# shangzhouye/stereo-visual-slam

Hardware: AMD Instinct MI355X
Metric: stereo keyframes/sec (ORB+match+tri+local-BA), KITTI-00 1241x376 (higher is better)
Workload: dtype u8+f64

## Files before the change

### stereo-visual-slam_amd/csrc/api.hip

```cpp
#include <stdarg.h>
#include <stdlib.h>

#include <algorithm>
#include <cmath>
#include <cfloat>
#include <vector>

#include "se3_device.h"
#include "vslam_internal.h"

#include <mutex>

namespace vslam {

static thread_local char g_err[512] = "";
void set_error(const char* fmt, ...) {
    va_list ap;
    va_start(ap, fmt);
    vsnprintf(g_err, sizeof(g_err), fmt, ap);
    va_end(ap);
}

struct Prof {
    struct Rec { const char* name; int launches; hipEvent_t e0, e1; };
// ... 33 lines not shown
        prof_set_current(((c)->prof && (c)->prof->on) ? (c)->prof : nullptr);               \
    } while (0)

int DevBuf::reserve(size_t need, hipStream_t stream) {
    if (bytes >= need) return VSLAM_OK;
    VS_HIP(hipStreamSynchronize(stream));
    release();
    const size_t want = std::max(need, min_bytes);
    if (hipMalloc((void**)&p, want) != hipSuccess) { p = nullptr; set_error("%s hipMalloc(%zu) failed", name, want); return VSLAM_ERR_HIP; }
    bytes = want; *acct += want;
    return VSLAM_OK;
}
void DevBuf::release() {
    if (p) { (void)hipFree(p); *acct -= bytes; }
    p = nullptr; bytes = 0;
}

struct Arena : Layout {
    struct Upload { void* d; const void* h; size_t bytes; };
    std::vector<Upload> uploads;
    explicit Arena(uint8_t* b = nullptr) : Layout(b) {}
    template <typename T> T* in(const T* h, size_t n) { T* d = take<T>(n); if (base) uploads.push_back({d, h, n * sizeof(T)}); return d; }
};
template <typename F>
static int arena_stage(Ctx* c, F&& layout) {
    Arena a;
    if (int rc = carve(c->stage, c->stream, a, layout)) return rc;
    for (const Arena::Upload& u : a.uploads) VS_HIP(hipMemcpyAsync(u.d, u.h, u.bytes, hipMemcpyHostToDevice, c->stream));
    return VSLAM_OK;
}

static CamParams cam_of(const Ctx* c) {
    CamParams cam;
    cam.fx = c->p.cam[0]; cam.fy = c->p.cam[1]; cam.cx = c->p.cam[2]; cam.cy = c->p.cam[3]; cam.b = c->p.cam[4];
    cam.dmin = c->p.depth_min; cam.dmax = c->p.depth_max; cam.drel = c->p.depth_reliable; cam.row_tol = c->p.stereo_row_tol;
    return cam;
}

template <typename T>
static int dev_alloc(Ctx* c, T** p, size_t n) {
    VS_HIP(hipMalloc((void**)p, n * sizeof(T)));
    c->dev_bytes += n * sizeof(T);
    return VSLAM_OK;
}

struct TuneKey { const char* name; const char* env; int Tuning::*field; int lo, hi; };
static const TuneKey kTuneKeys[] = {
    {"orb_fuse_min", "VSLAM_ORB_FUSE_MIN", &Tuning::orb_fuse_min, 0, 1 << 30},
    {"anms_cap", "VSLAM_ANMS_CAP", &Tuning::anms_cap, 0, 1 << 30},
    {"sgbm_fuse_min", "VSLAM_SGBM_FUSE_MIN", &Tuning::sgbm_fuse_min, 0, 1 << 30},
    {"sgbm_fwd_min", "VSLAM_SGBM_FWD_MIN", &Tuning::sgbm_fwd_min, 0, 1 << 30},
    {"sgbm_fw_rows", "VSLAM_SGBM_FW_ROWS", &Tuning::sgbm_fw_rows, 32, 64},
    {"pose_only_window", "VSLAM_POSE_ONLY_WINDOW", &Tuning::pose_only_window, 0, 1},
    {"ba_resident", "VSLAM_BA_RESIDENT", &Tuning::ba_resident, 0, 1},
    {"pnp_window", "VSLAM_PNP_WINDOW", &Tuning::pnp_window, 0, 1},
    {"ba_adaptive", "VSLAM_BA_ADAPTIVE", &Tuning::ba_adaptive, 0, 1},
    {"ba_lanes", "VSLAM_BA_LANES", &Tuning::ba_lanes, 256, 512},
    {"track_rule", "VSLAM_TRACK_RULE", &Tuning::track_rule, 0, 1},
    {"rectify_form", "VSLAM_RECTIFY_FORM", &Tuning::rectify_form, 0, 1},
};
static int tune_set(Tuning& t, const TuneKey& k, long v) {
    if (v == -1) { t.*(k.field) = -1; return VSLAM_OK; }
    if (v < k.lo || v > k.hi || (k.field == &Tuning::sgbm_fw_rows && v != 32 && v != 64) || (k.field == &Tuning::ba_lanes && v != 256 && v != 512)) {
        set_error("tuning value %s = %ld out of range (%d..%d%s, or -1 = default)", k.name, v, k.lo, k.hi, k.field == &Tuning::sgbm_fw_rows ? ", 32 or 64" : "");
        return VSLAM_ERR_ARG;
    }
    t.*(k.field) = (int)v;
    return VSLAM_OK;
}
static int tune_from_env(Tuning& t) {
    for (const TuneKey& k : kTuneKeys) {
        const char* e = getenv(k.env);
        if (!e || !*e) continue;
        char* end = nullptr;
        const long v = strtol(e, &end, 10);
        if (end == e || *end != 0) { set_error("environment variable %s = \"%s\" is not an integer", k.env, e); return VSLAM_ERR_ARG; }
        int rc = tune_set(t, k, v);
        if (rc) return rc;
    }
    return VSLAM_OK;
}

static int orb_status_check(Ctx* c, int B) {
    std::vector<int32_t> st(B);
    VS_HIP(hipMemcpyAsync(st.data(), c->orb.d_status, sizeof(int32_t) * B, hipMemcpyDeviceToHost, c->stream));
    VS_HIP(hipStreamSynchronize(c->stream));
    for (int b = 0; b < B; ++b)
        if (st[b]) { set_error("ORB capacity exceeded on image %d (status bits 0x%x)", b, st[b]); return VSLAM_ERR_CAPACITY; }
    return VSLAM_OK;
}

constexpr int kOrbFuseMinDefault = 96;
static int orb_fuse_min(const Ctx* c) { return c->tune.orb_fuse_min >= 0 ? c->tune.orb_fuse_min : kOrbFuseMinDefault; }

static int orb_pipeline(Ctx* c, const uint8_t* d_imgs, size_t img_bytes, int pitch, int B, int anms_num, int regroup, bool describe,
                        vslam_keypoint* d_kps, uint8_t* d_desc, int32_t* d_count) {
    if (B <= 0) return VSLAM_OK;
    if (B > c->p.max_batch) { set_error("batch %d exceeds context max_batch %d", B, c->p.max_batch); return VSLAM_ERR_ARG; }
    int rc;
    const bool fused = describe && B >= orb_fuse_min(c);
    if (fused) {
        if ((rc = launch_orb_pyrblur(c->plan, c->tab, d_imgs, img_bytes, pitch, B, c->orb.d_pyr, c->orb.d_blur, c->p.fast_threshold, c->orb.d_corners,
                                     c->orb.d_corner_cnt, c->orb.d_status, c->stream))) return rc;
    } else {
        if ((rc = launch_orb_pyramid(c->plan, c->tab, d_imgs, img_bytes, pitch, B, c->orb.d_pyr, c->stream))) return rc;
        if ((rc = launch_orb_fast(c->plan, d_imgs, img_bytes, pitch, B, c->orb.d_pyr, c->p.fast_threshold, c->orb.d_corners,
                                  c->orb.d_corner_cnt, c->orb.d_status, c->stream))) return rc;
    }
    if ((rc = launch_orb_select(c->plan, d_imgs, img_bytes, pitch, B, c->orb.d_pyr, c->orb.d_corners, c->orb.d_corner_cnt, c->orb.d_sel,
                                c->orb.d_sel_cnt, c->orb.d_status, c->stream))) return rc;
    if ((rc = launch_orb_anms(c->plan, B, c->orb.d_sel, c->orb.d_sel_cnt, c->plan.sel_cap, anms_num, regroup, d_kps, nullptr, c->orb.d_order, c->p.kp_capacity,
                              d_count, c->orb.d_status, c->orb.d_rad, c->tune.anms_cap, c->orb.d_anms_path, c->stream))) return rc;
    if ((rc = launch_orb_orient(c->plan, d_imgs, img_bytes, pitch, B, c->orb.d_pyr, d_kps, c->orb.d_cs, c->orb.d_order, c->p.kp_capacity, d_count, c->stream))) return rc;
    if (describe) {
        if (!fused && (rc = launch_orb_blur(c->plan, d_imgs, img_bytes, pitch, B, c->orb.d_pyr, c->orb.d_blur, c->stream))) return rc;
        if ((rc = launch_orb_describe(c->plan, d_imgs, img_bytes, pitch, B, c->orb.d_pyr, c->orb.d_blur, d_kps, c->orb.d_cs, c->orb.d_order, c->p.kp_capacity, d_count,
// ... 1408 lines not shown
```

### stereo-visual-slam_amd/csrc/lm_kernels.hip

```cpp
#include "vslam_internal.h"

#include <stdlib.h>

#include <vector>

#include "se3_device.h"
#include "lm_device.h"

namespace vslam {

constexpr int kLmBlock = 512;
constexpr int kLmItemFixed = 128;
constexpr int kLmMinWaves = 2;
constexpr int kLmWaves = kLmBlock / 64;
constexpr int kMaxKf = VSLAM_MAX_KF;
constexpr int kMaxNp = 6 * kMaxKf;
constexpr int kMaxPairs = kMaxKf * (kMaxKf + 1) / 2;
constexpr int kHitsPerEdge = (kMaxKf + 1) / 2 + 1;
constexpr int kDinvLds = 1950;
constexpr int kLin = 2;
constexpr int kPoseParts = 3;
constexpr int kCntStride = 80;
constexpr int kItemSlots = (kMaxPairs + kLmWaves - 1) / kLmWaves;
constexpr int kDbgSlots = 24;
// ... 1219 lines not shown
        while (again) {
            double x[6], E[7], Tt[7], Rtt[12], Hd[36], gd[6];
            const bool ok2 = chol6_solve(H, lambda, g, x);
            if (!ok2) {
#pragma unroll
                for (int i = 0; i < 6; ++i) x[i] = 0;
            }
            se3::exp(x, E);
            se3::mul(E, T, Tt);
            expand_pose(Tt, Rtt);
            double tempChi = evaluate(Rtt, false, Hd, gd);
            if (!ok2) tempChi = 1.7976931348623157e308;
            double scale = 1e-3;
#pragma unroll
            for (int i = 0; i < 6; ++i) scale += x[i] * (lambda * x[i] + g[i]);
            rho_gain = (currentChi - tempChi) / scale;
            if (rho_gain > 0 && isfinite(tempChi)) {
                double alpha = 1. - pow(2 * rho_gain - 1, 3);
                alpha = fmin(alpha, 2. / 3.);
                lambda *= fmax(1. / 3., alpha);
                ni = 2;
                currentChi = tempChi;
#pragma unroll
                for (int i = 0; i < 7; ++i) T[i] = Tt[i];
#pragma unroll
                for (int i = 0; i < 12; ++i) Rt[i] = Rtt[i];
            } else {
                lambda *= ni;
                ni *= 2;
            }
            ++qmax;
            again = (rho_gain < 0) && qmax < 10;
        }
        total_trials += qmax;
        if (st && lane == 0 && it < VSLAM_LM_MAX_ITERS) { st->chi2_iter[it] = currentChi; st->lambda_iter[it] = lambda; st->trials_iter[it] = qmax; }
        if (qmax == 10 || rho_gain == 0) { ++it; break; }
    }
    if (st && lane == 0) { st->iterations = it; st->total_trials = total_trials; st->chi2_final = currentChi; st->lambda_final = lambda; }
    if (lane < 7) d_T[7 * (size_t)b + lane] = T[lane];
    int mine = 0;
    for (int i = lane; i < n; i += 64) {
        const size_t gi = (size_t)b * capacity + i;
        double X, Y, Z, ex, ey;
        project_err(Rt, K, (double)px[3 * i], (double)px[3 * i + 1], (double)px[3 * i + 2], uv[2 * gi], uv[2 * gi + 1], X, Y, Z, ex, ey);
        const double c = ex * ex + ey * ey;
        const bool ok = isfinite(c) && c <= thr2;
        if (inlier) inlier[gi] = ok;
        mine += ok;
    }
    for (int o = 32; o > 0; o >>= 1) mine += __shfl_xor(mine, o);
    if (lane == 0 && n_inl) n_inl[b] = mine;
}

constexpr int kPoBlock = 64 * kMaxKf;
struct PoShared {
    double H[2][kMaxKf][36], g[2][kMaxKf][6];
    double part[2][kMaxKf], spart[2][kMaxKf];
    int cnt[kMaxKf][kMaxKf];
    int kbeg[kMaxKf + 1];
    int flag[2];
    int cin[2][kMaxKf], cout[2][kMaxKf];
    double T[2][kMaxKf][7], R[3][kMaxKf][12];
};
__global__ __launch_bounds__(kPoBlock) void pose_only_wave_kernel(LmKernelArgs ka, int iters, int update_poses) {
    const LmWindowArgs& a = ka.a;
    __shared__ PoShared sm;
    const int w = ka.order ? ka.order[blockIdx.x] : (int)blockIdx.x, tid = threadIdx.x, lane = tid & 63;
    const int wave = __builtin_amdgcn_readfirstlane(tid >> 6);
    if (ka.status[w] != VSLAM_OK) return;
    long long* cyc = ka.dbg_cycles ? ka.dbg_cycles + kDbgSlots * (size_t)w : nullptr;
    long long t_ph = cyc ? clock64() : 0;
#define POH(i) do { if (cyc && tid == 0) { const long long t1__ = clock64(); cyc[i] += t1__ - t_ph; t_ph = t1__; } } while (0)
    const int nk = a.n_kf_w ? min(max(a.n_kf_w[w], 1), a.n_kf) : a.n_kf;
    const int lm0 = a.lm_off[w], e0 = a.edge_off[w], ne = a.edge_off[w + 1] - e0;
    const int32_t* kfi = a.kf_idx + e0;
    const int32_t* lmi = a.lm_idx + e0;
    const float2* uv2 = reinterpret_cast<const float2*>(a.uv) + e0;
    const float* xyz = a.xyz + 3 * (size_t)lm0;
    uint8_t* inl = a.lm_inlier + lm0;
    int32_t* list = a.kf_edges + e0;
    float2* uvk = reinterpret_cast<float2*>(ka.uvk) + e0;
    float4* posk = reinterpret_cast<float4*>(a.lin) + e0;
    double* chik = ka.chi2k + e0;
    const double K[4] = {a.K[0], a.K[1], a.K[2], a.K[3]};
    const CamK ck = make_camk(K);
    const double delta = a.huber_delta;
    const unsigned long long lt_mask = (1ull << lane) - 1ull;
    const int per = (((ne + kMaxKf - 1) / kMaxKf) + 63) & ~63;
    const int c0 = min(wave * per, ne), c1 = min(c0 + per, ne);
    {
        int cnt[kMaxKf];
#pragma unroll
        for (int k = 0; k < kMaxKf; ++k) cnt[k] = 0;
        for (int base = c0; base < c1; base += 256) {
            int kq[4], lq[4]; bool vq[4]; uint8_t iq[4];
#pragma unroll
            for (int u = 0; u < 4; ++u) { const int e = base + 64 * u + lane; vq[u] = e < c1; const int es = min(e, ne - 1); kq[u] = kfi[es]; lq[u] = lmi[es]; }
#pragma unroll
            for (int u = 0; u < 4; ++u) iq[u] = inl[lq[u]];
#pragma unroll
            for (int u = 0; u < 4; ++u) {
                const bool act = vq[u] && iq[u] != 0;
#pragma unroll
                for (int kk = 0; kk < kMaxKf; ++kk) cnt[kk] += __popcll(__ballot(act && kq[u] == kk));
            }
        }
        if (lane < kMaxKf) {
            int v = 0;
#pragma unroll
            for (int kk = 0; kk < kMaxKf; ++kk) if (lane == kk) v = cnt[kk];
            sm.cnt[wave][lane] = v;
        }
        if (tid < 2) sm.flag[tid] = 0;
    }
    __syncthreads();
    int off[kMaxKf];
    {
        int run = 0;
#pragma unroll
        for (int k = 0; k < kMaxKf; ++k) {
            int before = 0, tot = 0;
#pragma unroll
            for (int c = 0; c < kMaxKf; ++c) { const int v = sm.cnt[c][k]; tot += v; if (c < wave) before += v; }
            off[k] = run + before;
            if (tid == 0) sm.kbeg[k] = run;
            run += tot;
        }
        if (tid == 0) sm.kbeg[kMaxKf] = run;
    }
    for (int base = c0; base < c1; base += 256) {
        int kq[4], lq[4], eq[4]; bool vq[4]; uint8_t iq[4]; float2 zq[4]; float Xq[4], Yq[4], Zq[4];
#pragma unroll
        for (int u = 0; u < 4; ++u) {
            const int e = base + 64 * u + lane; vq[u] = e < c1; eq[u] = e;
            const int es = min(e, ne - 1);
            kq[u] = kfi[es]; lq[u] = lmi[es]; zq[u] = uv2[es];
        }
#pragma unroll
        for (int u = 0; u < 4; ++u) { iq[u] = inl[lq[u]]; Xq[u] = xyz[3 * lq[u]]; Yq[u] = xyz[3 * lq[u] + 1]; Zq[u] = xyz[3 * lq[u] + 2]; }
#pragma unroll
        for (int u = 0; u < 4; ++u) {
            const bool act = vq[u] && iq[u] != 0;
#pragma unroll
            for (int kk = 0; kk < kMaxKf; ++kk) {
                const unsigned long long m = __ballot(act && kq[u] == kk);
                if (act && kq[u] == kk) {
                    const int pos = off[kk] + __popcll(m & lt_mask);
                    list[pos] = eq[u]; uvk[pos] = zq[u]; posk[pos] = make_float4(Xq[u], Yq[u], Zq[u], 0.f);
                }
                off[kk] += __popcll(m);
            }
        }
    }
    __syncthreads();
    POH(0);
    const int ntot = sm.kbeg[kMaxKf];
    const bool mine = wave < nk;
    const int kb = mine ? sm.kbeg[wave] : 0, ke = mine ? sm.kbeg[wave + 1] : 0;
    {
        double T[7], Rt[12];
#pragma unroll
        for (int i = 0; i < 7; ++i) T[i] = a.T[((size_t)w * a.n_kf + min(wave, nk - 1)) * 7 + i];
        expand_pose(T, Rt);
        if (lane == 0) {
#pragma unroll
            for (int i = 0; i < 7; ++i) sm.T[0][wave][i] = T[i];
#pragma unroll
            for (int i = 0; i < 12; ++i) { sm.R[0][wave][i] = Rt[i]; sm.R[2][wave][i] = Rt[i]; }
        }
        __builtin_amdgcn_wave_barrier();
    }
    const int slot27 = wave_slot<27>(lane);
    auto evaluate = [&](const double* Rlds, bool lin, int buf, bool store_chi) -> double {
        double R[12];
#pragma unroll
        for (int i = 0; i < 12; ++i) R[i] = uniform_f64(Rlds[i]);
        double part = 0, acc[27];
#pragma unroll
        for (int i = 0; i < 27; ++i) acc[i] = 0;
        float4 pp[2], pn[2]; float2 zz[2], zn[2];
#pragma unroll
        for (int u = 0; u < 2; ++u) { const int j = min(kb + 64 * u + lane, max(ke - 1, 0)); pp[u] = posk[j]; zz[u] = uvk[j]; }
        for (int j0 = kb; j0 < ke; j0 += 128) {
#pragma unroll
            for (int u = 0; u < 2; ++u) { const int j = min(j0 + 128 + 64 * u + lane, ke - 1); pn[u] = posk[j]; zn[u] = uvk[j]; }
#pragma unroll
            for (int u = 0; u < 2; ++u) {
                const int j = j0 + 64 * u + lane;
                if (j >= ke) continue;
                double x, y, ri, wgt, ex, ey, c, rho;
                cam_norm(R, (double)pp[u].x, (double)pp[u].y, (double)pp[u].z, x, y, ri);
                eval_obs(ck, x, y, zz[u], delta, ex, ey, c, rho, wgt);
                part += rho;
                if (store_chi) chik[j] = c;
                if (lin) {
                    double A[12], wA[12];
                    jac_norm(x, y, ri, A);
                    const double l0 = wgt * ck.fx2, l1 = wgt * ck.fy2;
#pragma unroll
                    for (int i = 0; i < 6; ++i) { wA[i] = l0 * A[i]; wA[6 + i] = l1 * A[6 + i]; }
                    int idx = 0;
#pragma unroll
                    for (int r = 0; r < 6; ++r)
#pragma unroll
                        for (int cc = r; cc < 6; ++cc) { acc[idx] = a_fma_pair(wA, r, A, cc, acc[idx]); ++idx; }
#pragma unroll
                    for (int r = 0; r < 6; ++r) acc[21 + r] = a_fma2(wA, r, -ex, -ey, acc[21 + r]);
                }
            }
#pragma unroll
            for (int u = 0; u < 2; ++u) { pp[u] = pn[u]; zz[u] = zn[u]; }
        }
        const double total = wave_sum(part);
        if (lin && mine) {
            wave_reduce_scatter<27>(acc, lane);
            if (slot27 >= 0 && slot27 < 21) {
                int r = 0, rem = slot27;
                while (rem >= 6 - r) { rem -= 6 - r; ++r; }
                const int cc = r + rem;
                sm.H[buf][wave][6 * r + cc] = acc[0]; sm.H[buf][wave][6 * cc + r] = acc[0];
            } else if (slot27 >= 21) sm.g[buf][wave][slot27 - 21] = acc[0];
        }
        return total;
    };
    auto sum_kf = [&](const double* v) -> double {
        double t = 0;
        for (int k = 0; k < nk; ++k) t += v[k];
        return t;
    };
    vslam_lm_stats* st = a.stats ? a.stats + w : nullptr;
    double lambda = 0, ni = 2, currentChi = 0;
    int pc = 0;
    int cur = 0, it = 0, total_trials = 0, pb = 0, fb = 0;
    if (iters > 0) {
        const double c = evaluate(sm.R[pc][wave], true, cur, false);
        if (lane == 0 && mine) sm.part[pb][wave] = c;
        __syncthreads();
        currentChi = sum_kf(sm.part[pb]);
        pb ^= 1;
        double md = 0;
        for (int k = 0; k < nk; ++k)
#pragma unroll
            for (int d = 0; d < 6; ++d) md = fmax(md, fabs(sm.H[cur][k][7 * d]));
        lambda = 1e-5 * md;
        if (st && tid == 0) st->chi2_init = currentChi;
    }
    POH(1);
    for (it = 0; it < iters; ++it) {
        double rho_gain = 0;
        int qmax = 0;
        bool again = true;
        while (again) {
            double x[6] = {0, 0, 0, 0, 0, 0};
            if (mine) {
                double Hk[36], gk[6];
#pragma unroll
                for (int i = 0; i < 36; ++i) Hk[i] = sm.H[cur][wave][i];
#pragma unroll
                for (int i = 0; i < 6; ++i) gk[i] = sm.g[cur][wave][i];
                if (!chol6_solve(Hk, lambda, gk, x) && lane == 0) sm.flag[fb] = 1;
            }
            POH(2);
            __syncthreads();
            POH(3);
            const bool ok2 = sm.flag[fb] == 0;
            if (tid == 0) sm.flag[fb ^ 1] = 0;
            fb ^= 1;
            if (!ok2) {
#pragma unroll
                for (int i = 0; i < 6; ++i) x[i] = 0;
            }
            {
                double E[7], Tc[7], Tt[7], Rtt[12];
#pragma unroll
                for (int i = 0; i < 7; ++i) Tc[i] = sm.T[pc][wave][i];
                se3::exp(x, E);
                se3::mul(E, Tc, Tt);
                expand_pose(Tt, Rtt);
                __builtin_amdgcn_wave_barrier();
                if (lane == 0) {
#pragma unroll
                    for (int i = 0; i < 7; ++i) sm.T[pc ^ 1][wave][i] = Tt[i];
#pragma unroll
                    for (int i = 0; i < 12; ++i) { sm.R[pc ^ 1][wave][i] = Rtt[i]; sm.R[2][wave][i] = Rtt[i]; }
                }
                __builtin_amdgcn_wave_barrier();
            }
            POH(4);
            const double c = evaluate(sm.R[pc ^ 1][wave], true, cur ^ 1, false);
            POH(5);
            double sc = 0;
            if (mine) {
#pragma unroll
                for (int i = 0; i < 6; ++i) sc += x[i] * (lambda * x[i] + sm.g[cur][wave][i]);
            }
            if (lane == 0 && mine) { sm.part[pb][wave] = c; sm.spart[pb][wave] = sc; }
            __syncthreads();
            POH(6);
            double tempChi = sum_kf(sm.part[pb]);
            const double scale = sum_kf(sm.spart[pb]) + 1e-3;
            pb ^= 1;
            if (!ok2) tempChi = 1.7976931348623157e308;
            rho_gain = (currentChi - tempChi) / scale;
            if (rho_gain > 0 && isfinite(tempChi)) {
                double alpha = 1. - pow(2 * rho_gain - 1, 3);
                alpha = fmin(alpha, 2. / 3.);
                lambda *= fmax(1. / 3., alpha);
                ni = 2;
                currentChi = tempChi;
                pc ^= 1;
                cur ^= 1;
            } else {
                lambda *= ni;
                ni *= 2;
            }
            ++qmax;
            again = (rho_gain < 0) && qmax < 10;
        }
        total_trials += qmax;
        if (st && tid == 0 && it < VSLAM_LM_MAX_ITERS) { st->chi2_iter[it] = currentChi; st->lambda_iter[it] = lambda; st->trials_iter[it] = qmax; }
        if (qmax == 10 || rho_gain == 0) { ++it; break; }
    }
    if (st && tid == 0) { st->iterations = it; st->total_trials = total_trials; st->chi2_final = currentChi; st->lambda_final = lambda; }
    POH(7);
    evaluate(sm.R[2][wave], false, 0, true);
    double th = delta;
    int cb = 0;
    for (int iteration = 0; iteration < 5; ++iteration) {
        int cin = 0, cout = 0;
        for (int j = kb + lane; j < ke; j += 64) { if (chik[j] > th) ++cout; else ++cin; }
        for (int o = 32; o > 0; o >>= 1) { cin += __shfl_xor(cin, o); cout += __shfl_xor(cout, o); }
        if (lane == 0) { sm.cin[cb][wave] = mine ? cin : 0; sm.cout[cb][wave] = mine ? cout : 0; }
        __syncthreads();
        int tin = 0, tout = 0;
        for (int k = 0; k < nk; ++k) { tin += sm.cin[cb][k]; tout += sm.cout[cb][k]; }
        cb ^= 1;
        const double ratio = (double)tin / (double)(tin + tout);
        if (ratio > 0.5) break;
        th *= 2;
    }
    if (ka.want_chi2) {
        double* chi2 = a.chi2 + e0;
        for (int e = tid; e < ne; e += kPoBlock) if (!inl[lmi[e]]) chi2[e] = 0.0;
        for (int j = kb + lane; j < ke; j += 64) chi2[list[j]] = chik[j];
    }
    __syncthreads();
    for (int j = kb + lane; j < ke; j += 64) {
        const int e = list[j];
        if (e == ne - 1 || lmi[e + 1] != lmi[e]) inl[lmi[e]] = !(chik[j] > th);
    }
    if (tid == 0 && a.chi2_thr) a.chi2_thr[w] = th;
    if (update_poses && mine && lane < 7) a.T[((size_t)w * a.n_kf + wave) * 7 + lane] = sm.T[pc][wave][lane];
    POH(8);
    (void)ntot;
#undef POH
}

static int carve_lm(LmScratch& s, LmKernelArgs& ka, size_t total_lm, size_t total_edge, int n_windows, bool with_lm, hipStream_t stream) {
    int32_t* defer;
    if (int rc = carve(s.buf, stream, [&](Layout& L) {
            ka.a.P = L.take<double>(total_lm * 3);
            ka.a.Ptrial = L.take<double>(total_lm * 3);
            ka.a.Hll = L.take<double>(total_lm * 6);
            ka.a.bl = L.take<double>(total_lm * 3);
            ka.a.Dinv = L.take<double>(total_lm * 6);
            ka.a.lin = L.take<double>(total_edge * kLin);
            ka.a.lm_ptr = L.take<int32_t>(total_lm + n_windows + 1);
            ka.a.kf_ptr = L.take<int32_t>((size_t)n_windows * (kMaxKf + 1));
            ka.a.kf_edges = L.take<int32_t>(total_edge);
            ka.a.pair_ptr = L.take<int32_t>((size_t)n_windows * (kMaxPairs + 1));
            ka.a.pair_hits = L.take<int32_t>(with_lm ? total_edge * kHitsPerEdge * 2 : 64);
            ka.act = L.take<uint8_t>(total_lm);
            ka.kf_pos = L.take<int32_t>(total_edge);
            ka.status = L.take<int32_t>(n_windows);
            double* chi2 = L.take<double>(total_edge);
            if (!ka.a.chi2) ka.a.chi2 = chi2;
            ka.chi2k = L.take<double>(total_edge);
            ka.uvk = L.take<float>(total_edge * 2);
            ka.slot_uv = L.take<float>(with_lm ? total_lm * kLmSlots * 2 : 64);
            ka.slot_kf = L.take<uint8_t>(with_lm ? total_lm * kLmSlots : 256);
            ka.lcnt = L.take<uint8_t>(total_lm);
            ka.order = L.take<int32_t>(n_windows);
            ka.passes = L.take<int32_t>(n_windows);
            defer = L.take<int32_t>(n_windows);
        })) return rc;
    s.status = ka.status; s.status_n = n_windows; s.passes = ka.passes; s.defer = defer;
    return VSLAM_OK;
}

__global__ void lm_fill_kernel(int32_t* __restrict__ p, int n, int v) { const int i = blockIdx.x * blockDim.x + threadIdx.x; if (i < n) p[i] = v; }
constexpr int kOrderCap = 4096;
__global__ __launch_bounds__(1024) void lm_order_kernel(const int32_t* __restrict__ edge_off, int n, int32_t* __restrict__ order) {
    __shared__ unsigned long long key[kOrderCap];
    int np2 = 1;
    while (np2 < n) np2 <<= 1;
    for (int i = threadIdx.x; i < np2; i += 1024)
        key[i] = i < n ? ((unsigned long long)(0xFFFFFFFFu - (unsigned)max(edge_off[i + 1] - edge_off[i], 0)) << 32) | (unsigned)i : ~0ull;
    for (int k = 2; k <= np2; k <<= 1)
        for (int j = k >> 1; j > 0; j >>= 1) {
            __syncthreads();
            for (int t = threadIdx.x; t < np2 / 2; t += 1024) {
                const int lo = ((t / j) * 2 * j) + (t % j), hi = lo + j;
                const bool up = (lo & k) == 0;
                const unsigned long long x = key[lo], y = key[hi];
                if ((x > y) == up) { key[lo] = y; key[hi] = x; }
            }
        }
// ... 24 lines not shown
        ka.dbg_cycles = (long long*)scratch->cyc.p;
    }
    int rc = carve_lm(*scratch, ka, total_lm, total_edge, a.n_windows, true, stream);
    if (rc) return rc;
    const bool adaptive = !(scratch->tune && scratch->tune->ba_adaptive == 0);
    const bool resident_on = (schedule || mode == 0) && !(scratch->tune && scratch->tune->ba_resident == 0);
    ProfScope prof__(stream, "lm_window_kernel", (schedule ? (adaptive ? 2 : 4) : 1) + (resident_on ? 1 : 0));
    if (a.n_windows > 1 && a.n_windows <= kOrderCap)
        hipLaunchKernelGGL(lm_order_kernel, dim3(1), dim3(1024), 0, stream, a.edge_off, a.n_windows, const_cast<int32_t*>(ka.order));
    else ka.order = nullptr;
    const bool resident = (schedule || mode == 0) && !(scratch->tune && scratch->tune->ba_resident == 0);
    scratch->defer_valid = resident;
    if (resident) {
        if (scratch->rs_dyn_bytes < 0) { int dev = 0; VS_HIP(hipGetDevice(&dev)); rs_query_device(dev, *scratch); }
        RsLaunch L;
        memset(&L, 0, sizeof(L));
        L.a = ka.a; L.uv_s = ka.uvk; L.epos = ka.kf_pos; L.tab = ka.a.Hll; L.xin = ka.a.Ptrial; L.Pbak = ka.a.P; L.Dc = ka.a.Dinv; L.blc = ka.a.bl;
        L.status = ka.status; L.passes = ka.passes; L.defer = scratch->defer; L.order = ka.order; L.dbg = getenv("VSLAM_RS_PROFILE") ? ka.dbg_cycles : nullptr;
        L.lanes = (scratch->tune && scratch->tune->ba_lanes > 0) ? scratch->tune->ba_lanes : 0;
        L.dyn_bytes = scratch->rs_dyn_bytes; L.full_bytes = scratch->rs_full_bytes; L.cu_count = scratch->rs_cu_count; L.schedule = schedule; L.adaptive = adaptive ? 1 : 0; L.iters = iters; L.update_poses = update_poses; L.update_lms = update_lms;
        L.opt_in_done = scratch->rs_opt_in; L.want_chi2 = ka.want_chi2;
        L.dense_to_general = !(scratch->tune && scratch->tune->ba_resident == 1);
        if (schedule && !adaptive) hipLaunchKernelGGL(lm_fill_kernel, dim3((a.n_windows + 255) / 256), dim3(256), 0, stream, ka.passes, a.n_windows, 3);
        rc = launch_ba_resident(L, stream);
        if (rc) return rc;
        scratch->rs_opt_in = true;
        ka.defer = scratch->defer;
        if (L.dbg) {
            hipStreamSynchronize(stream);
            std::vector<long long> h(kDbgSlots * (size_t)a.n_windows);
            hipMemcpy(h.data(), ka.dbg_cycles, sizeof(long long) * h.size(), hipMemcpyDeviceToHost);
            static const char* rs_names[16] = {"setup", "pass init", "boot evaluation", "lambda-init pass", "linearise", "convert+cholesky+solve", "pose update+backsub+trial eval",
                                               "(loop tail)", "classification", "write-back", "lin: row open", "lin: landmark blocks", "lin: diag pair (row-wise)", "lin: off-diag pairs (row-wise)", "lin: singles chunks", "(classification: row loop)"};
            double tot = 0;
            for (int i = 0; i < 16; ++i) { double sum = 0; for (int w = 0; w < a.n_windows; ++w) sum += (double)h[16 * (size_t)w + i]; sum /= a.n_windows; if (i < 10) tot += sum; fprintf(stderr, "  [rs profile] %-32s %10.0f ticks/window\n", rs_names[i], sum); }
            fprintf(stderr, "  [rs profile] total %.0f (clock64 ticks)\n", tot);
            hipMemsetAsync(ka.dbg_cycles, 0, sizeof(long long) * kDbgSlots * a.n_windows, stream);
        }
    }
    if (schedule) {
        if (adaptive) {
            hipLaunchKernelGGL((lm_window_kernel<false, true>), dim3(a.n_windows), dim3(kLmBlock), dyn_lds, stream, ka, 0, 5, 0, 0, 1, 0);
        } else {
            if (!resident) hipLaunchKernelGGL(lm_fill_kernel, dim3((a.n_windows + 255) / 256), dim3(256), 0, stream, ka.passes, a.n_windows, 3);
            hipLaunchKernelGGL(lm_window_kernel<false>, dim3(a.n_windows), dim3(kLmBlock), dyn_lds, stream, ka, 0, 5, 0, 0, 1, 0);
            hipLaunchKernelGGL(lm_window_kernel<false>, dim3(a.n_windows), dim3(kLmBlock), dyn_lds, stream, ka, 0, 5, 0, 0, 1, 1);
            hipLaunchKernelGGL(lm_window_kernel<false>, dim3(a.n_windows), dim3(kLmBlock), dyn_lds, stream, ka, 0, kSchedFinalIters, 1, 0, 1, 1);
        }
        ka.defer = nullptr;
        const bool po_window = scratch->tune && scratch->tune->pose_only_window > 0;
        if (po_window) hipLaunchKernelGGL(lm_window_kernel<false>, dim3(a.n_windows), dim3(kLmBlock), dyn_lds, stream, ka, 1, 10, 1, 0, 1, resident ? 0 : 1);
        else {
            if (ka.dbg_cycles && getenv("VSLAM_PO_PROFILE")) hipMemsetAsync(ka.dbg_cycles, 0, sizeof(long long) * kDbgSlots * a.n_windows, stream);
            hipLaunchKernelGGL(pose_only_wave_kernel, dim3(a.n_windows), dim3(kPoBlock), 0, stream, ka, 10, 1);
        }
    } else {
        hipLaunchKernelGGL(lm_window_kernel<false>, dim3(a.n_windows), dim3(kLmBlock), dyn_lds, stream, ka, mode, iters, update_poses, update_lms, 1, 0);
    }
    VS_HIP(hipGetLastError());
    if (ka.dbg_cycles) {
        hipStreamSynchronize(stream);
        std::vector<long long> h(kDbgSlots * (size_t)a.n_windows);
        hipMemcpy(h.data(), ka.dbg_cycles, sizeof(long long) * h.size(), hipMemcpyDeviceToHost);
        static const char* names[kDbgSlots] = {"setup", "eval+lin", "lm blocks", "pose blocks", "lambda/Dinv", "bs", "schur", "cholesky (rest)", "solve (rest)", "update+scale", "eval trial", "loop tail", "classify+wb", "(setup: csr)", "(setup: kf-major)", "schur: item prologue",
                                               "chol: diag+rows", "chol: barrier 1", "chol: trailing update", "chol: barrier 2", "solve: barrier", "solve: back-subst", "schur: rows", "schur: reduce+store"};
        double tot = 0;
        for (int i = 0; i < kDbgSlots; ++i) { double s = 0; for (int w = 0; w < a.n_windows; ++w) s += (double)h[kDbgSlots * (size_t)w + i]; s /= a.n_windows; if (i < 13 || i >= 16) tot += s; fprintf(stderr, "  [lm profile] %-20s %10.0f ticks/window\n", names[i], s); }
        fprintf(stderr, "  [lm profile] total %.0f cycles (clock64 = shader clock, thread 0 of every window; setup sub-splits not included)\n", tot);
    }
    return VSLAM_OK;
}

int lm_fetch_deferred(const LmScratch* scratch, int n_windows, int32_t* h_defer, hipStream_t stream) {
    if (!scratch->buf.p || !scratch->defer || !h_defer || n_windows > scratch->status_n) return VSLAM_ERR_ARG;
    if (!scratch->defer_valid) { for (int w = 0; w < n_windows; ++w) h_defer[w] = 1; return VSLAM_OK; }
    VS_HIP(hipMemcpyAsync(h_defer, scratch->defer, sizeof(int32_t) * n_windows, hipMemcpyDeviceToHost, stream));
    VS_HIP(hipStreamSynchronize(stream));
    for (int w = 0; w < n_windows; ++w) h_defer[w] &= 1;
    return VSLAM_OK;
}

int lm_fetch_passes(const LmScratch* scratch, int n_windows, int32_t* h_passes, hipStream_t stream) {
    if (!scratch->buf.p || !scratch->passes || !h_passes || n_windows > scratch->status_n) return VSLAM_ERR_ARG;
    VS_HIP(hipMemcpyAsync(h_passes, scratch->passes, sizeof(int32_t) * n_windows, hipMemcpyDeviceToHost, stream));
    VS_HIP(hipStreamSynchronize(stream));
    return VSLAM_OK;
}

int lm_fetch_status(const LmScratch* scratch, int n_windows, int32_t* h_status, hipStream_t stream) {
    const LmScratch& g_lm = *scratch;
    if (!g_lm.buf.p || !h_status) return VSLAM_ERR_ARG;
    VS_HIP(hipMemcpyAsync(h_status, g_lm.status, sizeof(int32_t) * n_windows, hipMemcpyDeviceToHost, stream));
    VS_HIP(hipStreamSynchronize(stream));
    return VSLAM_OK;
}

__global__ __launch_bounds__(256) void edge_jacobian_kernel(int n, const float* __restrict__ xyz, const float* __restrict__ uv, const double* __restrict__ T, double K0, double K1,
                                                           double K2, double K3, double delta, double* __restrict__ err, double* __restrict__ Jp, double* __restrict__ Jl,
                                                           double* __restrict__ chi2, double* __restrict__ hw) {
    const int i = blockIdx.x * 256 + threadIdx.x;
    if (i >= n) return;
    const double K[4] = {K0, K1, K2, K3};
    const CamK ck = make_camk(K);
    double Tl[7], Rt[12];
#pragma unroll
    for (int c = 0; c < 7; ++c) Tl[c] = T[c];
    expand_pose(Tl, Rt);
// ... 54 lines not shown
```

### stereo-visual-slam_amd/csrc/vslam_internal.h

```cpp
#pragma once
#include <hip/hip_runtime.h>
#include <stdint.h>
#include <stdio.h>
#include <string.h>

#include "../../include/vslam_hip.h"

namespace vslam {

void set_error(const char* fmt, ...);

#define VS_HIP(call)                                                                              \
    do {                                                                                          \
        hipError_t e__ = (call);                                                                  \
        if (e__ != hipSuccess) {                                                                  \
            ::vslam::set_error("%s:%d %s -> %s", __FILE__, __LINE__, #call, hipGetErrorString(e__)); \
            return VSLAM_ERR_HIP;                                                                 \
        }                                                                                         \
    } while (0)

struct Prof;
Prof* prof_current();
void prof_set_current(Prof* p);
void prof_begin(hipStream_t s, const char* name, int launches);
// ... 129 lines not shown
                 const int32_t* d_nt, const double* d_gap, int gate, double ratio, double gap_thr, int B, int max_rows,
                 uint32_t* d_train_best, vslam_dmatch* d_out, int out_capacity, int32_t* d_nout, hipStream_t stream,
                 const int32_t* d_qsel = nullptr, int sel_cap = 0, const int32_t* d_nqsel = nullptr, const int32_t* d_qitem = nullptr, int n_qitems = 0);

struct CamParams { double fx, fy, cx, cy, b, dmin, dmax, drel, row_tol; };
int launch_find3d_disparity(const vslam_keypoint* d_kps, int n, const float* d_disp, int w, int h, int dstride,
                            const double* d_T, CamParams cam, float* d_xyz, uint8_t* d_valid, uint8_t* d_rel, hipStream_t stream);
int launch_find3d_disparity_batch(const vslam_keypoint* d_kps, const int32_t* d_n, int kp_capacity, int B, const float* d_disp, int w, int h,
                                  const double* d_T, CamParams cam, float* d_xyz, uint8_t* d_valid, uint8_t* d_rel, hipStream_t stream);
int launch_triangulate(const float* d_uvL, const float* d_uvR, const int32_t* d_n, int capacity, int B, const double* d_T,
                       CamParams cam, float* d_xyz, uint8_t* d_valid, uint8_t* d_rel, hipStream_t stream);
int launch_build_pnp_inputs(const vslam_dmatch* d_m, const int32_t* d_nm, int match_capacity, const vslam_dmatch* d_lr,
                            const int32_t* d_nlr, int lr_capacity, const float* d_xyz_lr, const uint8_t* d_valid_lr,
                            const vslam_keypoint* d_kpsT, int kp_capacity, int B, int32_t* d_kp2lr, float* d_xyz_out, float* d_uv_out,
                            int32_t* d_nout, int out_capacity, hipStream_t stream);
int launch_gather_uv(const vslam_keypoint* d_kpsQ, const vslam_keypoint* d_kpsT, int kp_capacity, const vslam_dmatch* d_m,
                     const int32_t* d_nm, int match_capacity, int B, float* d_uvQ, float* d_uvT, hipStream_t stream);

int launch_hbm_copy_probe(const void* src, void* dst, size_t bytes, int variant, hipStream_t stream);
int hbm_copy_probe_variants();
const char* hbm_copy_probe_name(int variant);

struct LmWindowArgs {
    int n_windows, n_kf;
    const int32_t* n_kf_w;
    const int32_t* lm_off;
    const int32_t* edge_off;
    double* T;
    float* xyz;
    const uint8_t* reliable;
    uint8_t* lm_inlier;
    const int32_t* kf_idx;
    const int32_t* lm_idx;
    const float* uv;
    double* chi2;
    vslam_lm_stats* stats;
    double* P;
    double* Ptrial;
    double* Hll;
    double* bl;
    double* Dinv;
    double* lin;
    int32_t* lm_ptr;
    int32_t* kf_ptr;
    int32_t* kf_edges;
    int32_t* pair_ptr;
    int32_t* pair_hits;
    int32_t hit_capacity_per_edge;
    double K[4];
    double huber_delta;
    double* chi2_thr;
    size_t total_lm, total_edge;
};
struct Tuning {
    int orb_fuse_min = -1;
    int anms_cap = -1;
    int sgbm_fuse_min = -1;
    int sgbm_fwd_min = -1;
    int sgbm_fw_rows = -1;
    int pose_only_window = -1;
    int pnp_window = -1;
    int ba_lanes = -1;
    int ba_resident = -1;
    int track_rule = -1;
    int rectify_form = -1;
    int ba_adaptive = -1;
};
constexpr int kSgbmTicketPools = 8;
constexpr int kSgbmErrorWord = kSgbmTicketPools;
int launch_sgbm(const Tuning& tune, const vslam_sgbm_params& sp, const uint8_t* d_left, const uint8_t* d_right, size_t img_bytes, int pitch, int w, int h, int B,
                float* d_disp_f32, int16_t* d_disp_i16, int16_t* d_disp_raw, DevBuf& scratch, hipStream_t stream);

struct LmScratch {
    DevBuf buf, cyc;
    int32_t* status = nullptr; int status_n = 0;
    int32_t* passes = nullptr;
    const Tuning* tune = nullptr;
    bool lds_opt_in = false;
    bool rs_opt_in = false;
    int rs_dyn_bytes = -1, rs_full_bytes = 0, rs_cu_count = 0;
    int32_t* defer = nullptr;
    bool defer_valid = false;
    explicit LmScratch(size_t* acct) : buf("LM scratch", acct), cyc("LM clock buffer", acct) {}
};
struct RsLaunch {
    LmWindowArgs a;
    void* uv_s; int32_t* epos; double* tab; double* xin; double* Pbak; double* Dc; double* blc;
    int32_t* status; int32_t* passes; int32_t* defer; const int32_t* order; long long* dbg;
    int dyn_bytes, full_bytes, cu_count;
    int schedule, adaptive, iters, update_poses, update_lms, dense_to_general;
    int want_chi2;
    int lanes;
    bool opt_in_done;
};
void rs_query_device(int device, LmScratch& s);
int launch_ba_resident(const RsLaunch& L, hipStream_t stream);
int launch_lm_windows(const LmWindowArgs& a, int schedule, int mode, int iters, int update_poses, int update_lms, LmScratch* scratch,
                      hipStream_t stream);
size_t lm_hits_per_edge();
int lm_fetch_status(const LmScratch* scratch, int n_windows, int32_t* h_status, hipStream_t stream);
int lm_fetch_passes(const LmScratch* scratch, int n_windows, int32_t* h_passes, hipStream_t stream);
int lm_fetch_deferred(const LmScratch* scratch, int n_windows, int32_t* h_defer, hipStream_t stream);

struct PnpArgs {
    const float* xyz; const float* uv; const int32_t* n; int capacity; int B;
    double* T; int iters; double K[4]; double huber_delta; double reproj_thr;
    uint8_t* inlier; int32_t* n_inliers; vslam_lm_stats* stats;
    int n_hint;
};
int launch_pnp(const PnpArgs& a, LmScratch* scratch, hipStream_t stream);
int launch_edge_jacobians(int n, const float* d_xyz, const float* d_uv, const double* d_T, const double K[4], double delta, double* d_err, double* d_Jp, double* d_Jl,
                          double* d_chi2, double* d_hw, hipStream_t stream);
size_t pnp_epnp_ws_bytes(int H);
// ... 61 lines not shown
```

Measured before the change: 64550.

## Add narrow pose-only kernel variant packing several keyframes per wave

The pose-only refinement kernel is templated on the wave count, so one block can run with fewer waves than keyframes. When a block has fewer waves, keyframes are dealt greedily by edge count, and each wave loops over its held keyframes. Solved steps pass through shared memory between waves. The host picks the narrow four-wave variant when there are more windows than CUs, which aims to raise occupancy and cut idle waves, at the cost of serialising work inside each wave. The wide variant also gets a min-waves launch bound of 3.

```diff
diff --git a/stereo-visual-slam_amd/csrc/api.hip b/stereo-visual-slam_amd/csrc/api.hip
--- a/stereo-visual-slam_amd/csrc/api.hip
+++ b/stereo-visual-slam_amd/csrc/api.hip
@@ -109,6 +109,7 @@
     {"sgbm_fwd_min", "VSLAM_SGBM_FWD_MIN", &Tuning::sgbm_fwd_min, 0, 1 << 30},
     {"sgbm_fw_rows", "VSLAM_SGBM_FW_ROWS", &Tuning::sgbm_fw_rows, 32, 64},
     {"pose_only_window", "VSLAM_POSE_ONLY_WINDOW", &Tuning::pose_only_window, 0, 1},
+    {"pose_only_waves", "VSLAM_POSE_ONLY_WAVES", &Tuning::pose_only_waves, 0, VSLAM_MAX_KF},
     {"ba_resident", "VSLAM_BA_RESIDENT", &Tuning::ba_resident, 0, 1},
     {"pnp_window", "VSLAM_PNP_WINDOW", &Tuning::pnp_window, 0, 1},
     {"ba_adaptive", "VSLAM_BA_ADAPTIVE", &Tuning::ba_adaptive, 0, 1},
@@ -118,7 +119,8 @@
 };
 static int tune_set(Tuning& t, const TuneKey& k, long v) {
     if (v == -1) { t.*(k.field) = -1; return VSLAM_OK; }
-    if (v < k.lo || v > k.hi || (k.field == &Tuning::sgbm_fw_rows && v != 32 && v != 64) || (k.field == &Tuning::ba_lanes && v != 256 && v != 512)) {
+    if (v < k.lo || v > k.hi || (k.field == &Tuning::sgbm_fw_rows && v != 32 && v != 64) || (k.field == &Tuning::ba_lanes && v != 256 && v != 512) ||
+        (k.field == &Tuning::pose_only_waves && v != 0 && v != VSLAM_MAX_KF && v != kPoseOnlyNarrowWaves)) {
         set_error("tuning value %s = %ld out of range (%d..%d%s, or -1 = default)", k.name, v, k.lo, k.hi, k.field == &Tuning::sgbm_fw_rows ? ", 32 or 64" : "");
         return VSLAM_ERR_ARG;
     }
diff --git a/stereo-visual-slam_amd/csrc/lm_kernels.hip b/stereo-visual-slam_amd/csrc/lm_kernels.hip
--- a/stereo-visual-slam_amd/csrc/lm_kernels.hip
+++ b/stereo-visual-slam_amd/csrc/lm_kernels.hip
@@ -1295,17 +1295,20 @@
     if (lane == 0 && n_inl) n_inl[b] = mine;
 }
 
-constexpr int kPoBlock = 64 * kMaxKf;
 struct PoShared {
     double H[2][kMaxKf][36], g[2][kMaxKf][6];
     double part[2][kMaxKf], spart[2][kMaxKf];
+    double x[kMaxKf][6];
     int cnt[kMaxKf][kMaxKf];
     int kbeg[kMaxKf + 1];
     int flag[2];
     int cin[2][kMaxKf], cout[2][kMaxKf];
     double T[2][kMaxKf][7], R[3][kMaxKf][12];
 };
-__global__ __launch_bounds__(kPoBlock) void pose_only_wave_kernel(LmKernelArgs ka, int iters, int update_poses) {
+template <int W, int kMinWaves>
+__global__ __launch_bounds__(64 * W, kMinWaves) void pose_only_wave_kernel(LmKernelArgs ka, int iters, int update_poses) {
+    static_assert(W == kMaxKf || (W >= 1 && W <= 8), "the keyframe deal takes its minimum over eight lanes");
+    constexpr int kBlock = 64 * W;
     const LmWindowArgs& a = ka.a;
     __shared__ PoShared sm;
     const int w = ka.order ? ka.order[blockIdx.x] : (int)blockIdx.x, tid = threadIdx.x, lane = tid & 63;
@@ -1329,7 +1332,7 @@
     const CamK ck = make_camk(K);
     const double delta = a.huber_delta;
     const unsigned long long lt_mask = (1ull << lane) - 1ull;
-    const int per = (((ne + kMaxKf - 1) / kMaxKf) + 63) & ~63;
+    const int per = (((ne + W - 1) / W) + 63) & ~63;
     const int c0 = min(wave * per, ne), c1 = min(c0 + per, ne);
     {
         int cnt[kMaxKf];
@@ -1364,7 +1367,7 @@
         for (int k = 0; k < kMaxKf; ++k) {
             int before = 0, tot = 0;
 #pragma unroll
-            for (int c = 0; c < kMaxKf; ++c) { const int v = sm.cnt[c][k]; tot += v; if (c < wave) before += v; }
+            for (int c = 0; c < W; ++c) { const int v = sm.cnt[c][k]; tot += v; if (c < wave) before += v; }
             off[k] = run + before;
             if (tid == 0) sm.kbeg[k] = run;
             run += tot;
@@ -1397,24 +1400,44 @@
     }
     __syncthreads();
     POH(0);
-    const int ntot = sm.kbeg[kMaxKf];
-    const bool mine = wave < nk;
-    const int kb = mine ? sm.kbeg[wave] : 0, ke = mine ? sm.kbeg[wave + 1] : 0;
-    {
+    unsigned long long held = 0;
+    int nheld = 0;
+    if constexpr (W == kMaxKf) { held = (unsigned long long)wave; nheld = wave < nk ? 1 : 0; }
+    else {
+        const int kl = min(lane, kMaxKf - 1);
+        const int mycnt = lane < nk ? sm.kbeg[kl + 1] - sm.kbeg[kl] : -1;
+        int rank = 0;
+        for (int j = 0; j < nk; ++j) { const int cj = sm.kbeg[j + 1] - sm.kbeg[j]; rank += (cj > mycnt || (cj == mycnt && j < lane)) ? 1 : 0; }
+        int load = 0;
+        for (int r = 0; r < nk; ++r) {
+            const int k = __builtin_amdgcn_readfirstlane(__ffsll((long long)__ballot(lane < nk && rank == r)) - 1);
+            const int cr = __shfl(mycnt, k);
+            int key = lane < W ? load * 16 + lane : 0x7fffffff;
+            key = min(key, __shfl_xor(key, 1)); key = min(key, __shfl_xor(key, 2)); key = min(key, __shfl_xor(key, 4));
+            const int v = __builtin_amdgcn_readfirstlane(key) & 15;
+            if (lane == v) load += cr;
+            if (v == wave) { held |= (unsigned long long)k << (4 * nheld); ++nheld; }
+        }
+    }
+    auto kf_at = [&](int q) -> int { return (int)((held >> (4 * q)) & 15ull); };
+#pragma unroll 1
+    for (int q = 0; q < nheld; ++q) {
+        const int k = kf_at(q);
         double T[7], Rt[12];
 #pragma unroll
-        for (int i = 0; i < 7; ++i) T[i] = a.T[((size_t)w * a.n_kf + min(wave, nk - 1)) * 7 + i];
+        for (int i = 0; i < 7; ++i) T[i] = a.T[((size_t)w * a.n_kf + k) * 7 + i];
         expand_pose(T, Rt);
         if (lane == 0) {
 #pragma unroll
-            for (int i = 0; i < 7; ++i) sm.T[0][wave][i] = T[i];
-#pragma unroll
-            for (int i = 0; i < 12; ++i) { sm.R[0][wave][i] = Rt[i]; sm.R[2][wave][i] = Rt[i]; }
-        }
-        __builtin_amdgcn_wave_barrier();
-    }
+            for (int i = 0; i < 7; ++i) sm.T[0][k][i] = T[i];
+#pragma unroll
+            for (int i = 0; i < 12; ++i) { sm.R[0][k][i] = Rt[i]; sm.R[2][k][i] = Rt[i]; }
+        }
+    }
+    __builtin_amdgcn_wave_barrier();
     const int slot27 = wave_slot<27>(lane);
-    auto evaluate = [&](const double* Rlds, bool lin, int buf, bool store_chi) -> double {
+    auto evaluate = [&](const double* Rlds, bool lin, int buf, bool store_chi, int k) -> double {
+        const int kb = __builtin_amdgcn_readfirstlane(sm.kbeg[k]), ke = __builtin_amdgcn_readfirstlane(sm.kbeg[k + 1]);
         double R[12];
 #pragma unroll
         for (int i = 0; i < 12; ++i) R[i] = uniform_f64(Rlds[i]);
@@ -1455,14 +1478,14 @@
             for (int u = 0; u < 2; ++u) { pp[u] = pn[u]; zz[u] = zn[u]; }
         }
         const double total = wave_sum(part);
-        if (lin && mine) {
+        if (lin) {
             wave_reduce_scatter<27>(acc, lane);
             if (slot27 >= 0 && slot27 < 21) {
                 int r = 0, rem = slot27;
                 while (rem >= 6 - r) { rem -= 6 - r; ++r; }
                 const int cc = r + rem;
-                sm.H[buf][wave][6 * r + cc] = acc[0]; sm.H[buf][wave][6 * cc + r] = acc[0];
-            } else if (slot27 >= 21) sm.g[buf][wave][slot27 - 21] = acc[0];
+                sm.H[buf][k][6 * r + cc] = acc[0]; sm.H[buf][k][6 * cc + r] = acc[0];
+            } else if (slot27 >= 21) sm.g[buf][k][slot27 - 21] = acc[0];
         }
         return total;
     };
@@ -1476,8 +1499,12 @@
     int pc = 0;
     int cur = 0, it = 0, total_trials = 0, pb = 0, fb = 0;
     if (iters > 0) {
-        const double c = evaluate(sm.R[pc][wave], true, cur, false);
-        if (lane == 0 && mine) sm.part[pb][wave] = c;
+#pragma unroll 1
+        for (int q = 0; q < nheld; ++q) {
+            const int k = kf_at(q);
+            const double c = evaluate(sm.R[pc][k], true, cur, false, k);
+            if (lane == 0) sm.part[pb][k] = c;
+        }
         __syncthreads();
         currentChi = sum_kf(sm.part[pb]);
         pb ^= 1;
@@ -1494,14 +1521,23 @@
         int qmax = 0;
         bool again = true;
         while (again) {
-            double x[6] = {0, 0, 0, 0, 0, 0};
-            if (mine) {
-                double Hk[36], gk[6];
-#pragma unroll
-                for (int i = 0; i < 36; ++i) Hk[i] = sm.H[cur][wave][i];
-#pragma unroll
-                for (int i = 0; i < 6; ++i) gk[i] = sm.g[cur][wave][i];
+            double xw[6] = {0, 0, 0, 0, 0, 0};
+#pragma unroll 1
+            for (int q = 0; q < nheld; ++q) {
+                const int k = kf_at(q);
+                double Hk[36], gk[6], x[6] = {0, 0, 0, 0, 0, 0};
+#pragma unroll
+                for (int i = 0; i < 36; ++i) Hk[i] = sm.H[cur][k][i];
+#pragma unroll
+                for (int i = 0; i < 6; ++i) gk[i] = sm.g[cur][k][i];
                 if (!chol6_solve(Hk, lambda, gk, x) && lane == 0) sm.flag[fb] = 1;
+                if constexpr (W == kMaxKf) {
+#pragma unroll
+                    for (int i = 0; i < 6; ++i) xw[i] = x[i];
+                } else if (lane == 0) {
+#pragma unroll
+                    for (int i = 0; i < 6; ++i) sm.x[k][i] = x[i];
+                }
             }
             POH(2);
             __syncthreads();
@@ -1509,35 +1545,35 @@
             const bool ok2 = sm.flag[fb] == 0;
             if (tid == 0) sm.flag[fb ^ 1] = 0;
             fb ^= 1;
-            if (!ok2) {
-#pragma unroll
-                for (int i = 0; i < 6; ++i) x[i] = 0;
-            }
-            {
-                double E[7], Tc[7], Tt[7], Rtt[12];
-#pragma unroll
-                for (int i = 0; i < 7; ++i) Tc[i] = sm.T[pc][wave][i];
-                se3::exp(x, E);
-                se3::mul(E, Tc, Tt);
-                expand_pose(Tt, Rtt);
-                __builtin_amdgcn_wave_barrier();
-                if (lane == 0) {
-#pragma unroll
-                    for (int i = 0; i < 7; ++i) sm.T[pc ^ 1][wave][i] = Tt[i];
-#pragma unroll
-                    for (int i = 0; i < 12; ++i) { sm.R[pc ^ 1][wave][i] = Rtt[i]; sm.R[2][wave][i] = Rtt[i]; }
-                }
-                __builtin_amdgcn_wave_barrier();
-            }
-            POH(4);
-            const double c = evaluate(sm.R[pc ^ 1][wave], true, cur ^ 1, false);
-            POH(5);
-            double sc = 0;
-            if (mine) {
-#pragma unroll
-                for (int i = 0; i < 6; ++i) sc += x[i] * (lambda * x[i] + sm.g[cur][wave][i]);
-            }
-            if (lane == 0 && mine) { sm.part[pb][wave] = c; sm.spart[pb][wave] = sc; }
+#pragma unroll 1
+            for (int q = 0; q < nheld; ++q) {
+                const int k = kf_at(q);
+                double sc = 0;
+                {
+                    double x[6], E[7], Tc[7], Tt[7], Rtt[12];
+#pragma unroll
+                    for (int i = 0; i < 6; ++i) x[i] = !ok2 ? 0.0 : W == kMaxKf ? xw[i] : sm.x[k][i];
+#pragma unroll
+                    for (int i = 0; i < 6; ++i) sc += x[i] * (lambda * x[i] + sm.g[cur][k][i]);
+#pragma unroll
+                    for (int i = 0; i < 7; ++i) Tc[i] = sm.T[pc][k][i];
+                    se3::exp(x, E);
+                    se3::mul(E, Tc, Tt);
+                    expand_pose(Tt, Rtt);
+                    __builtin_amdgcn_wave_barrier();
+                    if (lane == 0) {
+#pragma unroll
+                        for (int i = 0; i < 7; ++i) sm.T[pc ^ 1][k][i] = Tt[i];
+#pragma unroll
+                        for (int i = 0; i < 12; ++i) { sm.R[pc ^ 1][k][i] = Rtt[i]; sm.R[2][k][i] = Rtt[i]; }
+                    }
+                    __builtin_amdgcn_wave_barrier();
+                }
+                POH(4);
+                const double c = evaluate(sm.R[pc ^ 1][k], true, cur ^ 1, false, k);
+                POH(5);
+                if (lane == 0) { sm.part[pb][k] = c; sm.spart[pb][k] = sc; }
+            }
             __syncthreads();
             POH(6);
             double tempChi = sum_kf(sm.part[pb]);
@@ -1566,14 +1602,19 @@
     }
     if (st && tid == 0) { st->iterations = it; st->total_trials = total_trials; st->chi2_final = currentChi; st->lambda_final = lambda; }
     POH(7);
-    evaluate(sm.R[2][wave], false, 0, true);
+#pragma unroll 1
+    for (int q = 0; q < nheld; ++q) { const int k = kf_at(q); evaluate(sm.R[2][k], false, 0, true, k); }
     double th = delta;
     int cb = 0;
     for (int iteration = 0; iteration < 5; ++iteration) {
-        int cin = 0, cout = 0;
-        for (int j = kb + lane; j < ke; j += 64) { if (chik[j] > th) ++cout; else ++cin; }
-        for (int o = 32; o > 0; o >>= 1) { cin += __shfl_xor(cin, o); cout += __shfl_xor(cout, o); }
-        if (lane == 0) { sm.cin[cb][wave] = mine ? cin : 0; sm.cout[cb][wave] = mine ? cout : 0; }
+#pragma unroll 1
+        for (int q = 0; q < nheld; ++q) {
+            const int k = kf_at(q), kb = sm.kbeg[k], ke = sm.kbeg[k + 1];
+            int cin = 0, cout = 0;
+            for (int j = kb + lane; j < ke; j += 64) { if (chik[j] > th) ++cout; else ++cin; }
+            for (int o = 32; o > 0; o >>= 1) { cin += __shfl_xor(cin, o); cout += __shfl_xor(cout, o); }
+            if (lane == 0) { sm.cin[cb][k] = cin; sm.cout[cb][k] = cout; }
+        }
         __syncthreads();
         int tin = 0, tout = 0;
         for (int k = 0; k < nk; ++k) { tin += sm.cin[cb][k]; tout += sm.cout[cb][k]; }
@@ -1584,18 +1625,25 @@
     }
     if (ka.want_chi2) {
         double* chi2 = a.chi2 + e0;
-        for (int e = tid; e < ne; e += kPoBlock) if (!inl[lmi[e]]) chi2[e] = 0.0;
-        for (int j = kb + lane; j < ke; j += 64) chi2[list[j]] = chik[j];
+        for (int e = tid; e < ne; e += kBlock) if (!inl[lmi[e]]) chi2[e] = 0.0;
+#pragma unroll 1
+        for (int q = 0; q < nheld; ++q) {
+            const int k = kf_at(q), kb = sm.kbeg[k], ke = sm.kbeg[k + 1];
+            for (int j = kb + lane; j < ke; j += 64) chi2[list[j]] = chik[j];
+        }
     }
     __syncthreads();
-    for (int j = kb + lane; j < ke; j += 64) {
-        const int e = list[j];
-        if (e == ne - 1 || lmi[e + 1] != lmi[e]) inl[lmi[e]] = !(chik[j] > th);
+#pragma unroll 1
+    for (int q = 0; q < nheld; ++q) {
+        const int k = kf_at(q), kb = sm.kbeg[k], ke = sm.kbeg[k + 1];
+        for (int j = kb + lane; j < ke; j += 64) {
+            const int e = list[j];
+            if (e == ne - 1 || lmi[e + 1] != lmi[e]) inl[lmi[e]] = !(chik[j] > th);
+        }
+        if (update_poses && lane < 7) a.T[((size_t)w * a.n_kf + k) * 7 + lane] = sm.T[pc][k][lane];
     }
     if (tid == 0 && a.chi2_thr) a.chi2_thr[w] = th;
-    if (update_poses && mine && lane < 7) a.T[((size_t)w * a.n_kf + wave) * 7 + lane] = sm.T[pc][wave][lane];
     POH(8);
-    (void)ntot;
 #undef POH
 }
 
@@ -1726,7 +1774,14 @@
         if (po_window) hipLaunchKernelGGL(lm_window_kernel<false>, dim3(a.n_windows), dim3(kLmBlock), dyn_lds, stream, ka, 1, 10, 1, 0, 1, resident ? 0 : 1);
         else {
             if (ka.dbg_cycles && getenv("VSLAM_PO_PROFILE")) hipMemsetAsync(ka.dbg_cycles, 0, sizeof(long long) * kDbgSlots * a.n_windows, stream);
-            hipLaunchKernelGGL(pose_only_wave_kernel, dim3(a.n_windows), dim3(kPoBlock), 0, stream, ka, 10, 1);
+            if (scratch->rs_dyn_bytes < 0) { int dev = 0; VS_HIP(hipGetDevice(&dev)); rs_query_device(dev, *scratch); }
+            const int forced = scratch->tune ? scratch->tune->pose_only_waves : -1;
+            const int waves = forced > 0 ? forced : (a.n_windows <= scratch->rs_cu_count ? kMaxKf : kPoseOnlyNarrowWaves);
+            switch (waves) {
+            case kMaxKf: hipLaunchKernelGGL((pose_only_wave_kernel<kMaxKf, 3>), dim3(a.n_windows), dim3(64 * kMaxKf), 0, stream, ka, 10, 1); break;
+            case kPoseOnlyNarrowWaves: hipLaunchKernelGGL((pose_only_wave_kernel<kPoseOnlyNarrowWaves, 2>), dim3(a.n_windows), dim3(64 * kPoseOnlyNarrowWaves), 0, stream, ka, 10, 1); break;
+            default: set_error("pose_only_waves %d is not built", waves); return VSLAM_ERR_ARG;
+            }
         }
     } else {
         hipLaunchKernelGGL(lm_window_kernel<false>, dim3(a.n_windows), dim3(kLmBlock), dyn_lds, stream, ka, mode, iters, update_poses, update_lms, 1, 0);
diff --git a/stereo-visual-slam_amd/csrc/vslam_internal.h b/stereo-visual-slam_amd/csrc/vslam_internal.h
--- a/stereo-visual-slam_amd/csrc/vslam_internal.h
+++ b/stereo-visual-slam_amd/csrc/vslam_internal.h
@@ -205,6 +205,7 @@
     double* chi2_thr;
     size_t total_lm, total_edge;
 };
+constexpr int kPoseOnlyNarrowWaves = 4;
 struct Tuning {
     int orb_fuse_min = -1;
     int anms_cap = -1;
@@ -212,6 +213,7 @@
     int sgbm_fwd_min = -1;
     int sgbm_fw_rows = -1;
     int pose_only_window = -1;
+    int pose_only_waves = -1;
     int pnp_window = -1;
     int ba_lanes = -1;
     int ba_resident = -1;
```

After: 67900, median of 6. 1.05x the previous value.
